# linnanwang/FastGen

Hardware: AMD Instinct MI355X
Metric: images/sec at 4-step distilled (DMD2) sampling (higher is better)
Workload: dtype fp32 (tensors, accumulate) with split-bf16 x3 MFMA conv products; 1 GPU; EDM CIFAR-10 32x32 SongUNet (55.7M params) DMD2 4-step 'sde' sampling, batch=512 per GPU; global_batch=512, sample_steps=4, parallelism=replicas x1 (no data-path collective), graph=True

## Files before the change

fastgen_amd/_lib.py:

```python
import ctypes
import os
from ctypes import POINTER, c_char_p, c_double, c_float, c_int, c_int64, c_size_t, c_uint64, c_void_p

_HERE = os.path.dirname(os.path.abspath(__file__))
LIB_PATH = os.path.join(_HERE, "libfastgen_amd.so")

FG_MAX_LEVELS = 8
FG_DTYPE_F32, FG_DTYPE_BF16, FG_DTYPE_BF16X3 = 0, 1, 2
DTYPE_NAMES = {"fp32": FG_DTYPE_F32, "bf16": FG_DTYPE_BF16, "bf16x3": FG_DTYPE_BF16X3}
FG_SAMPLE_SDE, FG_SAMPLE_ODE = 0, 1
FG_LOOP_X0, FG_LOOP_MEANFLOW, FG_LOOP_EULER = 0, 1, 2
FG_SCHEDULE_EDM, FG_SCHEDULE_RF = 0, 1
FG_DROP_PRECOND_INPUT, FG_DROP_PRECOND_OUTPUT = 1, 2
FG_BWD_DECODER, FG_BWD_ENCODER, FG_BWD_EMBED = 1, 2, 4
FG_MODEL_SONGUNET, FG_MODEL_DHARIWAL = 0, 1


class fg_edm_config(ctypes.Structure):
    _fields_ = [
        ("img_resolution", c_int), ("img_channels", c_int), ("label_dim", c_int), ("augment_dim", c_int),
        ("model_channels", c_int), ("num_levels", c_int), ("channel_mult", c_int * FG_MAX_LEVELS),
        ("channel_mult_emb", c_int), ("num_blocks", c_int), ("num_attn_resolutions", c_int),
        ("attn_resolutions", c_int * FG_MAX_LEVELS), ("channel_mult_noise", c_int), ("sigma_data", c_double),
        ("sigma_shift", c_double), ("compute_dtype", c_int), ("r_timestep", c_int), ("drop_precond", c_int),
# ... 9 lines not shown
        ("concat_balance", c_double), ("res_balance", c_double), ("attn_balance", c_double), ("clip_act", c_double),
        ("sigma_data", c_double), ("sigma_shift", c_double), ("compute_dtype", c_int), ("drop_precond", c_int),
    ]


class fg_dit_config(ctypes.Structure):
    _fields_ = [("input_size", c_int), ("patch_size", c_int), ("in_channels", c_int), ("hidden_size", c_int), ("depth", c_int),
                ("num_heads", c_int), ("mlp_hidden", c_int), ("embedding_rows", c_int), ("r_timestep", c_int), ("compute_dtype", c_int)]


class fg_wan_config(ctypes.Structure):
    _fields_ = [("num_heads", c_int), ("head_dim", c_int), ("in_channels", c_int), ("out_channels", c_int), ("text_dim", c_int),
                ("freq_dim", c_int), ("ffn_dim", c_int), ("num_layers", c_int), ("rope_max_seq_len", c_int), ("chunk_size", c_int),
                ("total_num_frames", c_int), ("eps", c_float)]


class fg_dit_sampler_config(ctypes.Structure):
    _fields_ = [("t_scale", c_double), ("guidance_scale", c_double), ("use_sit_convention", c_int), ("time_cond_diff", c_int),
                ("net_pred_flow", c_int), ("schedule", c_int)]


class fg_wan_sampler_config(ctypes.Structure):
    _fields_ = [("t_scale", c_double), ("context_noise", c_double), ("net_pred_flow", c_int), ("schedule", c_int), ("prefill_frames", c_int)]


SIGNATURES = {
    "fg_last_error": (c_char_p, []),
    "fg_version": (c_char_p, []),
    "fg_edm_create": (c_int, [POINTER(fg_edm_config), POINTER(c_void_p)]),
    "fg_edm_destroy": (None, [c_void_p]),
    "fg_edm_num_params": (c_int, [c_void_p]),
    "fg_edm_param_info": (c_int, [c_void_p, c_int, POINTER(c_char_p), POINTER(c_int), POINTER(c_int64)]),
    "fg_edm_bind_param": (c_int, [c_void_p, c_char_p, c_void_p, c_int64]),
    "fg_edm_pack_weights": (c_int, [c_void_p, c_void_p]),
    "fg_edm_workspace_bytes": (c_size_t, [c_void_p, c_int]),
    "fg_edm_forward": (c_int, [c_void_p, c_void_p, c_void_p, c_void_p, c_void_p, c_void_p, c_void_p, c_int, c_void_p,
                               c_size_t, c_void_p]),
    "fg_edm_num_feature_taps": (c_int, [c_void_p]),
    "fg_edm_feature_info": (c_int, [c_void_p, c_int, POINTER(c_char_p), POINTER(c_int), POINTER(c_int)]),
    "fg_edm_forward_features": (c_int, [c_void_p, c_void_p, c_void_p, c_void_p, c_void_p, c_void_p, POINTER(c_void_p), c_int,
                                        c_void_p, c_size_t, c_void_p]),
    "fg_sampler_run": (c_int, [c_void_p, c_void_p, c_void_p, POINTER(c_double), c_int, c_int, c_int, c_void_p, c_uint64,
                               c_void_p, c_int, c_void_p, c_size_t, c_int, c_void_p]),
    "fg_edm_t_list": (c_int, [c_int, POINTER(c_double)]),
    "fg_rf_t_list": (c_int, [c_int, POINTER(c_double)]),
    "fg_edm_profile_begin": (c_int, [c_void_p]),
    "fg_edm_profile_end": (c_int, [c_void_p, POINTER(c_int64), POINTER(c_double), POINTER(c_double)]),
    "fg_edm_num_blocks": (c_int, [c_void_p]),
    "fg_edm_block_info": (c_int, [c_void_p, c_int, POINTER(c_char_p), POINTER(c_int), POINTER(c_int), POINTER(c_int),
                                  POINTER(c_int), POINTER(c_int)]),
    "fg_edm_run_block": (c_int, [c_void_p, c_int, c_void_p, c_int, c_void_p, c_int, c_void_p, c_void_p, c_int, c_void_p,
                                 c_size_t, c_void_p]),
    "fg_op_gn_coeffs": (c_int, [c_void_p, c_int, c_void_p, c_int, c_void_p, c_void_p, c_float, c_void_p, c_int, c_int, c_void_p]),
    "fg_op_adm_conv_pack_bytes": (c_size_t, [c_int, c_int, c_int, c_int]),
    "fg_op_adm_conv_pack": (c_int, [c_int, c_void_p, c_void_p, c_int, c_int, c_int, c_void_p]),
    "fg_op_adm_conv": (c_int, [c_int, c_int, c_void_p, c_int, c_void_p, c_int, c_int, c_int, c_int, c_int, c_void_p, c_int, c_void_p,
                               c_void_p, c_void_p, c_int, c_void_p, c_int, c_void_p]),
    "fg_op_adm_gn_workspace_bytes": (c_size_t, [c_int, c_int, c_int]),
    "fg_op_adm_gn_coeffs": (c_int, [c_void_p, c_int, c_void_p, c_int, c_void_p, c_void_p, c_float, c_void_p, c_int, c_void_p, c_int,
                                    c_int, c_void_p, c_size_t, c_void_p]),
    "fg_op_adm_attention": (c_int, [c_void_p, c_void_p, c_int, c_int, c_int, c_void_p]),
    "fg_op_adm_map_in": (c_int, [c_void_p, c_void_p, c_void_p, c_void_p, c_int, c_void_p, c_int, c_int, c_void_p]),
    "fg_op_latents": (c_int, [c_void_p, c_double, c_void_p, c_int64, c_void_p]),
    "fg_op_forward_process": (c_int, [c_void_p, c_void_p, c_double, c_int, c_void_p, c_int64, c_void_p]),
    "fg_op_x0_to_eps": (c_int, [c_void_p, c_void_p, c_double, c_int, c_void_p, c_int64, c_void_p]),
    "fg_op_conv_wgrad_workspace_bytes": (ctypes.c_size_t, [c_int, c_int, c_int, c_int, c_int]),
    "fg_op_conv_wgrad": (c_int, [c_void_p, c_void_p, c_void_p, c_int, c_int, c_int, c_int, c_int, c_int, c_void_p, ctypes.c_size_t, c_void_p]),
    "fg_op_conv_wgrad_f32": (c_int, [c_void_p, c_void_p, c_void_p, c_int, c_int, c_int, c_int, c_int, c_int, c_void_p, ctypes.c_size_t, c_void_p]),
    "fg_edm_bind_grad": (c_int, [c_void_p, c_char_p, c_void_p, c_int64]),
    "fg_edm_block_backward_workspace_bytes": (c_size_t, [c_void_p, c_int, c_int]),
    "fg_edm_run_block_backward": (c_int, [c_void_p, c_int, c_void_p, c_int, c_void_p, c_int, c_void_p, c_void_p, c_void_p,
                                          c_void_p, c_void_p, c_int, c_void_p, c_size_t, c_void_p]),
    "fg_edm_backward_workspace_bytes": (c_size_t, [c_void_p, c_int]),
    "fg_edm_backward": (c_int, [c_void_p, c_void_p, c_void_p, c_void_p, c_void_p, c_void_p, c_void_p, c_int, c_int, c_void_p,
                                c_size_t, c_void_p]),
    "fg_edm_forward_train": (c_int, [c_void_p, c_void_p, c_void_p, c_void_p, c_void_p, c_void_p, c_void_p, c_int, c_void_p,
                                     c_size_t, c_void_p]),
    "fg_edm_backward_ex": (c_int, [c_void_p, c_void_p, c_void_p, c_void_p, c_void_p, c_void_p, c_void_p, c_void_p, c_void_p, c_int,
                                   c_int, c_void_p, c_size_t, c_void_p]),
    "fg_edm_backward_part": (c_int, [c_void_p, c_void_p, c_void_p, c_void_p, c_void_p, c_void_p, c_void_p, c_void_p, c_void_p, c_int,
                                     c_int, c_int, c_void_p, c_size_t, c_void_p]),
    "fg_edm2_create": (c_int, [POINTER(fg_edm2_config), POINTER(c_void_p)]),
    "fg_edm2_destroy": (None, [c_void_p]),
    "fg_edm2_num_params": (c_int, [c_void_p]),
    "fg_edm2_param_info": (c_int, [c_void_p, c_int, POINTER(c_char_p), POINTER(c_int), POINTER(c_int64)]),
    "fg_edm2_bind_param": (c_int, [c_void_p, c_char_p, c_void_p, c_int64]),
    "fg_edm2_pack_weights": (c_int, [c_void_p, c_void_p]),
    "fg_edm2_workspace_bytes": (c_size_t, [c_void_p, c_int]),
    "fg_edm2_forward": (c_int, [c_void_p, c_void_p, c_void_p, c_void_p, c_void_p, c_void_p, c_int, c_void_p, c_size_t, c_void_p]),
    "fg_edm2_set_training": (c_int, [c_void_p, c_int]),
    "fg_edm2_sampler_run": (c_int, [c_void_p, c_void_p, c_void_p, POINTER(c_double), c_int, c_int, c_int, c_void_p, c_uint64,
                                    c_void_p, c_int, c_void_p, c_size_t, c_int, c_void_p]),
    "fg_edm2_num_blocks": (c_int, [c_void_p]),
    "fg_edm2_block_info": (c_int, [c_void_p, c_int, POINTER(c_char_p), POINTER(c_int), POINTER(c_int), POINTER(c_int),
                                   POINTER(c_int), POINTER(c_int)]),
    "fg_edm2_run_block": (c_int, [c_void_p, c_int, c_void_p, c_int, c_void_p, c_int, c_void_p, c_void_p, c_int, c_void_p,
                                  c_size_t, c_void_p]),
    "fg_dit_create": (c_int, [POINTER(fg_dit_config), POINTER(c_void_p)]),
    "fg_dit_destroy": (None, [c_void_p]),
    "fg_dit_num_params": (c_int, [c_void_p]),
    "fg_dit_param_info": (c_int, [c_void_p, c_int, POINTER(c_char_p), POINTER(c_int), POINTER(c_int64)]),
    "fg_dit_bind_param": (c_int, [c_void_p, c_char_p, c_void_p, c_int64]),
    "fg_dit_pack_weights": (c_int, [c_void_p, c_void_p]),
    "fg_dit_pack_group": (c_int, [c_void_p, c_char_p, c_char_p, c_void_p]),
    "fg_dit_workspace_bytes": (c_size_t, [c_void_p, c_int]),
    "fg_dit_forward": (c_int, [c_void_p, c_void_p, c_void_p, c_void_p, c_void_p, c_void_p, c_void_p, c_int, c_void_p, c_size_t, c_void_p]),
# ... 66 lines not shown
```

fastgen_amd/csrc/conv.h:

```cpp
#pragma once
#include <hip/hip_runtime.h>

struct ConvArgs {
    const void* src1;
    const void* src2;
    int C1, C2;
    int Hs, Ws;
    int H, W;
    int B;
    const float2* ab;
    const void* wpack;
    const void* wpack_ws;
    const float* bias;
    const float* temb;
    int temb_stride;
    const void* resid;
    float scale;
    void* out;
    int Cout;
    float2* stats;
    int dbg;
    void* q_out;
    void* k_out;
    void* vt_out;
    const float* gate = nullptr;
    int gate_stride = 0;
    int act = 0;
    int heads = 0, head_dim = 0;
    size_t heads_lo_off = 0;
};

enum { PRO_NONE = 0, PRO_GN = 1, PRO_GN_SILU = 2 };
enum { RES_NONE = 0, RES_DOWN = 1, RES_UP = 2 };
enum { OUT_NHWC = 0, OUT_QKV = 1, OUT_TOK = 2, OUT_HEADS = 3 };

int launch_conv_fused(int dtype, int ks, int pro, int res, int outmode, const ConvArgs& a, hipStream_t stream);
int conv_stat_slots(int W);
bool conv_ws_supported(int dtype, int ks, int pro, int res, int outmode, const ConvArgs& a);
bool conv_ws_enabled();
int launch_conv_ws(int res, const ConvArgs& a, hipStream_t stream, bool prepare_only, int pro = PRO_GN_SILU);
bool conv_ws_shape_ok(int dtype, int cout, int cin, int res);
int launch_pack_conv_weights_ws(const float* w_oihw, void* wpack_ws, int cout, int cin, hipStream_t stream);
bool conv_x3ws_supported(int ks, int pro, int res, int outmode, const ConvArgs& a);
bool conv_x3ws_shape_ok(int cout, int cin, int res);
int conv_x3ws_stat_slots(int W);
int launch_conv_x3ws(int res, const ConvArgs& a, hipStream_t stream, bool prepare_only, int pro = PRO_GN_SILU);
int launch_pack_conv_weights_x3ws(const float* w_oihw, void* wpack_ws, int cout, int cin, hipStream_t stream);
int conv_launch_stat_slots(int dtype, int ks, int pro, int res, int outmode, const ConvArgs& a);
int launch_conv_ws_debug(const ConvArgs& a, int abl, hipStream_t stream);
int launch_conv_debug(int dtype, const ConvArgs& a, hipStream_t stream);
int conv_prepare_all(int dtype);
size_t conv_pack_elems(int cout, int cin, int ks);
int launch_pack_conv_weights(int dtype, const float* w_oihw, void* wpack, int cout, int cin, int ks, int qkv_perm,
                             hipStream_t stream);
```

fastgen_amd/csrc/conv.hip:

```cpp
#include "common.h"
#include "conv.h"
#include <stdlib.h>

#include <type_traits>

namespace {

constexpr int PITCH = 144;
constexpr int NTHR = 256;

template <int KS, int LOGW>
struct Geom {
    static constexpr int W = 1 << LOGW;
    static constexpr int LOGTW = (LOGW == 5) ? 4 : LOGW;
    static constexpr int TW = 1 << LOGTW;
    static constexpr int LOGTH = 3;
    static constexpr int TH = 1 << LOGTH;
    static constexpr int IMGS = 128 / (TH * TW);
    static constexpr int TCOLS = W / TW;
    static constexpr int TPI = (IMGS > 1) ? 1 : (W / TH) * TCOLS;
    static constexpr int PAD = KS / 2;
    static constexpr int HW_ = TW + 2 * PAD;
    static constexpr int HH_ = TH + 2 * PAD;
    static constexpr int HALO_PIX = IMGS * HH_ * HW_;
// ... 527 lines not shown
        if (res == RES_UP) return launch_w<T, 3, PRO_GN_SILU, RES_UP, OUT_NHWC>(a, s);
    }
    if (ks == 3 && pro == PRO_NONE && res == RES_NONE) return launch_w<T, 3, PRO_NONE, RES_NONE, OUT_NHWC>(a, s);
    if (ks == 1 && pro == PRO_NONE) {
        if (res == RES_NONE) return launch_w<T, 1, PRO_NONE, RES_NONE, OUT_NHWC>(a, s);
        if (res == RES_DOWN) return launch_w<T, 1, PRO_NONE, RES_DOWN, OUT_NHWC>(a, s);
        if (res == RES_UP) return launch_w<T, 1, PRO_NONE, RES_UP, OUT_NHWC>(a, s);
    }
    return (int)hipErrorInvalidValue;
}

int dispatch_t(int dtype, int ks, int pro, int res, int outmode, const ConvArgs& a, hipStream_t s) {
    switch (dtype) {
        case 0: return launch_t<float>(ks, pro, res, outmode, a, s);
        case 1: return launch_t<__bf16>(ks, pro, res, outmode, a, s);
        case 2: return launch_t<bf16x3>(ks, pro, res, outmode, a, s);
    }
    return (int)hipErrorInvalidValue;
}

}

int launch_conv_debug(int dtype, const ConvArgs& a, hipStream_t stream) {
    if (dtype != 1 || a.W != 32) return (int)hipErrorInvalidValue;
    g_debug_extra_lds = (a.dbg & 16) ? 48 * 1024 : 0;
    switch (a.dbg & 15) {
        case 0: return launch_one<__bf16, 3, PRO_GN_SILU, RES_NONE, 5, OUT_NHWC, 0>(a, stream);
        case 1: return launch_one<__bf16, 3, PRO_GN_SILU, RES_NONE, 5, OUT_NHWC, 1>(a, stream);
        case 2: return launch_one<__bf16, 3, PRO_GN_SILU, RES_NONE, 5, OUT_NHWC, 2>(a, stream);
        case 3: return launch_one<__bf16, 3, PRO_GN_SILU, RES_NONE, 5, OUT_NHWC, 3>(a, stream);
        case 4: return launch_one<__bf16, 3, PRO_GN_SILU, RES_NONE, 5, OUT_NHWC, 4>(a, stream);
        case 5: return launch_one<__bf16, 3, PRO_GN_SILU, RES_NONE, 5, OUT_NHWC, 5>(a, stream);
        case 6: return launch_one<__bf16, 3, PRO_GN_SILU, RES_NONE, 5, OUT_NHWC, 6>(a, stream);
        case 7: return launch_one<__bf16, 3, PRO_GN_SILU, RES_NONE, 5, OUT_NHWC, 7>(a, stream);
    }
    return (int)hipErrorInvalidValue;
}

int launch_conv_fused(int dtype, int ks, int pro, int res, int outmode, const ConvArgs& a, hipStream_t stream) {
    const int kc = dtype == 1 ? DT<__bf16>::KC : DT<float>::KC;
    if (a.H != a.W || (a.W != 8 && a.W != 16 && a.W != 32)) return (int)hipErrorInvalidValue;
    const bool tok = outmode == OUT_TOK || outmode == OUT_HEADS;
    if ((a.C1 % kc) || (a.C2 % kc) || (a.Cout % (tok ? 64 : 256)) || a.B <= 0) return (int)hipErrorInvalidValue;
    if (outmode == OUT_HEADS && (a.heads <= 0 || (a.head_dim % 4) || a.Cout != 3 * a.heads * a.head_dim || ((a.heads * a.head_dim) % 64) ||
                                 !a.q_out || !a.k_out || !a.vt_out))
        return (int)hipErrorInvalidValue;
    if (res == RES_NONE && (a.Hs != a.H || a.Ws != a.W)) return (int)hipErrorInvalidValue;
    if (res == RES_DOWN && (a.Hs != 2 * a.H || a.Ws != 2 * a.W)) return (int)hipErrorInvalidValue;
    if (res == RES_UP && (2 * a.Hs != a.H || 2 * a.Ws != a.W)) return (int)hipErrorInvalidValue;
    if (pro != PRO_NONE && !a.ab) return (int)hipErrorInvalidValue;
    if (outmode == OUT_QKV && (a.Cout != 768 || a.W > 16)) return (int)hipErrorInvalidValue;
    if (conv_ws_enabled() && conv_ws_supported(dtype, ks, pro, res, outmode, a)) return launch_conv_ws(res, a, stream, false, pro);
    if (dtype == 2 && conv_ws_enabled() && conv_x3ws_supported(ks, pro, res, outmode, a)) return launch_conv_x3ws(res, a, stream, false, pro);
    return dispatch_t(dtype, ks, pro, res, outmode, a, stream);
}

bool conv_ws_enabled() {
    static const bool on = [] {
        const char* e = getenv("FASTGEN_AMD_CONV_WS");
        return !(e && e[0] == '0');
    }();
    return on;
}

int conv_launch_stat_slots(int dtype, int ks, int pro, int res, int outmode, const ConvArgs& a) {
    if (dtype == 2 && conv_ws_enabled() && conv_x3ws_supported(ks, pro, res, outmode, a)) return conv_x3ws_stat_slots(a.W);
    return conv_stat_slots(a.W);
}

int conv_stat_slots(int W) { return W == 32 ? Geom<3, 5>::TPI : (W == 16 ? Geom<3, 4>::TPI : Geom<3, 3>::TPI); }

int conv_prepare_all(int dtype) {
    g_prepare_only = true;
    int rc = 0;
    ConvArgs a{};
    a.B = 1;
    a.Cout = 256;
    const int ws[3] = {8, 16, 32};
    for (int wi = 0; wi < 3 && !rc; ++wi) {
        a.W = a.H = ws[wi];
        for (int res = 0; res < 3 && !rc; ++res) {
            if (res != RES_DOWN)
                rc = dispatch_t(dtype, 3, PRO_GN_SILU, res, OUT_NHWC, a, nullptr);
            if (!rc) rc = dispatch_t(dtype, 1, PRO_NONE, res, OUT_NHWC, a, nullptr);
        }
        if (!rc) rc = dispatch_t(dtype, 3, PRO_NONE, RES_NONE, OUT_NHWC, a, nullptr);
        if (!rc && a.W <= 16) rc = dispatch_t(dtype, 1, PRO_GN, RES_NONE, OUT_QKV, a, nullptr);
        if (!rc && a.W == 16) rc = dispatch_t(dtype, 1, PRO_NONE, RES_NONE, OUT_TOK, a, nullptr);
        if (!rc && a.W == 16) rc = dispatch_t(dtype, 1, PRO_NONE, RES_NONE, OUT_HEADS, a, nullptr);
    }
    g_prepare_only = false;
    if (!rc && dtype == 2) {
        ConvArgs w{};
        for (int res : {RES_NONE, RES_UP})
            for (int ww : {32, 16}) {
                w.W = w.H = ww;
                if (!rc) rc = launch_conv_x3ws(res, w, nullptr, true, PRO_GN_SILU);
                if (!rc && res == RES_NONE) rc = launch_conv_x3ws(res, w, nullptr, true, PRO_NONE);
            }
    }
    if (!rc && dtype == 1) {
        ConvArgs w{};
        for (int res : {RES_NONE, RES_UP}) {
            w.W = w.H = 32;
            if (!rc) rc = launch_conv_ws(res, w, nullptr, true);
            if (res == RES_NONE) {
                w.C1 = -128;
                if (!rc) rc = launch_conv_ws(res, w, nullptr, true);
                w.C1 = 0;
            }
            w.W = w.H = 16;
            if (!rc) rc = launch_conv_ws(res, w, nullptr, true);
        }
    }
    return rc;
}

size_t conv_pack_elems(int cout, int cin, int ks) { return (size_t)cout * cin * ks * ks; }

// ... 13 lines not shown
```

fastgen_amd/csrc/engine.hip:

```cpp
#include <hip/hip_runtime.h>

#include <cmath>
#include <cstdarg>
#include <cstdio>
#include <cstdlib>
#include <cstring>
#include <string>
#include <map>
#include <vector>

#include "../../include/fastgen_amd.h"
#include "common.h"
#include "adm.h"
#include "edm2.h"
#include "conv.h"
#include "misc.h"

namespace {

thread_local std::string g_err;

int fail(int code, const char* fmt, ...) {
    char buf[512];
    va_list ap;
// ... 1183 lines not shown
}

int fg_edm_run_block(fg_edm* h, int index, const float* x1, int c1, const float* x2, int c2, const float* emb, float* out,
                     int batch, void* workspace, size_t workspace_bytes, void* stream) {
    if (!h || !x1 || !emb || !out) return fail(FG_EINVAL, "null argument");
    if (h->adm) return adm_run_block(h, index, x1, c1, x2, c2, emb, out, batch, workspace, workspace_bytes, (hipStream_t)stream);
    if (!h->packed) return fail(FG_ENOTREADY, "weights are not packed (call fg_edm_pack_weights)");
    if (index < 0 || index >= (int)h->blocks.size()) return fail(FG_EINVAL, "block index out of range");
    Workspace w;
    int rc0 = setup_ws(plan_workspace, h, batch, workspace, workspace_bytes, w);
    if (rc0) return rc0;
    hipStream_t s = (hipStream_t)stream;
    HIP_TRY(launch_linear(emb, h->aff_w, h->aff_b, w.temb, batch, h->emb_ch, h->temb_total, 0, s));
    const Block& b = *h->blocks[index];
    const size_t npix_in = (size_t)batch * b.res_in * b.res_in, npix_out = (size_t)batch * b.res_out * b.res_out;
    Act a1, a2;
    HIP_TRY(launch_to_act(h->dtype, x1, w.cvt1, (int64_t)npix_in * c1, s));
    a1.p = w.cvt1;
    if (c2) {
        HIP_TRY(launch_to_act(h->dtype, x2, w.cvt2, (int64_t)npix_in * c2, s));
        a2.p = w.cvt2;
    }
    int rc = run_block(h, b, a1, c1, a2, c2, w.temb, w.xa, batch, w, s);
    if (rc) return rc;
    HIP_TRY(launch_from_act(h->dtype, w.xa.p, out, (int64_t)npix_out * b.cout, s));
    return FG_OK;
}

#include "engine_train.inc"
#include "engine_dit.inc"
#include "engine_wan.inc"
#include "engine_sampler.inc"
#include "engine_edm2.inc"

int fg_op_gn_coeffs(const float* x1, int c1, const float* x2, int c2, const float* gamma, const float* beta, float eps,
                    float* ab_out, int batch, int hw, void* stream) {
    if (!x1 || !gamma || !beta || !ab_out) return fail(FG_EINVAL, "null argument");
    HIP_TRY(launch_gn_coeffs(0, x1, c1, c2 ? x2 : nullptr, c2, gamma, beta, eps, (float2*)ab_out, batch, hw, (hipStream_t)stream));
    return FG_OK;
}

size_t fg_op_adm_conv_pack_bytes(int mode, int cout, int cin, int ks) {
    if ((mode != FG_DTYPE_BF16 && mode != FG_DTYPE_BF16X3) || (ks != 1 && ks != 3) || cout <= 0 || cin <= 0 || cin % 32) return 0;
    return adm_conv_pack_elems(mode, cout, cin, ks) * sizeof(__bf16);
}
int fg_op_adm_conv_pack(int mode, const float* w_oihw, void* packed, int cout, int cin, int ks, void* stream) {
    if (!fg_op_adm_conv_pack_bytes(mode, cout, cin, ks))
        return fail(FG_EINVAL, "fg_op_adm_conv_pack: mode %d (1 bf16, 2 bf16x3), ks %d (1, 3), cout %d > 0, cin %d (multiple of 32)", mode,
                    ks, cout, cin);
    if (!w_oihw || !packed) return fail(FG_EINVAL, "fg_op_adm_conv_pack: null pointer");
    HIP_TRY(adm_pack_conv_weights(mode, w_oihw, packed, cout, cin, ks, (hipStream_t)stream));
    return FG_OK;
}
int fg_op_adm_conv(int mode, int ks, const float* src1, int c1, const float* src2, int c2, int batch, int hs, int h, int res_mode,
                   const float* ab, int silu, const void* packed, const float* bias, const float* resid, int resid_mode, float* out,
                   int cout, void* stream) {
    if ((mode != FG_DTYPE_BF16 && mode != FG_DTYPE_BF16X3) || (ks != 1 && ks != 3))
        return fail(FG_EINVAL, "fg_op_adm_conv: mode %d (1 bf16, 2 bf16x3), ks %d (1, 3)", mode, ks);
    if (c1 <= 0 || c1 % 32 || c2 < 0 || c2 % 32 || cout <= 0 || batch <= 0 || batch > 65535)
        return fail(FG_EINVAL, "fg_op_adm_conv: c1 %d > 0 and c2 %d >= 0 multiples of 32, cout %d > 0, batch %d in 1 .. 65535", c1, c2,
                    cout, batch);
    const bool res_ok = (res_mode == 0 && hs == h) || (res_mode == 1 && hs == 2 * h) || (res_mode == 2 && h == 2 * hs);
    if (h <= 0 || h > 4096 || !res_ok) return fail(FG_EINVAL, "fg_op_adm_conv: res_mode %d with hs %d, h %d", res_mode, hs, h);
    if (resid && (resid_mode < 0 || resid_mode > 2 || (resid_mode == 2 && h % 2)))
        return fail(FG_EINVAL, "fg_op_adm_conv: resid_mode %d (0, 1, 2 with h even) at h %d", resid_mode, h);
    if (!src1 || (c2 && !src2) || !packed || !out) return fail(FG_EINVAL, "fg_op_adm_conv: null pointer");
    if (((uintptr_t)src1 | (uintptr_t)(c2 ? src2 : nullptr) | (uintptr_t)packed) & 15 || (uintptr_t)ab & 7)
        return fail(FG_EINVAL, "fg_op_adm_conv: src1 / src2 / packed must be 16-byte aligned, ab 8-byte aligned");
    AdmConvArgs a;
    a.src1 = src1, a.src2 = c2 ? src2 : nullptr, a.C1 = c1, a.C2 = c2, a.Hs = hs, a.H = h, a.B = batch, a.res_mode = res_mode;
    a.ab = (const float2*)ab, a.silu = silu ? 1 : 0, a.w = packed, a.bias = bias, a.resid = resid, a.resid_mode = resid ? resid_mode : 0;
    a.out = out, a.Cout = cout;
    HIP_TRY(adm_launch_conv(mode, ks, a, (hipStream_t)stream));
    return FG_OK;
}
size_t fg_op_adm_gn_workspace_bytes(int batch, int hw, int c) {
    if (batch <= 0 || hw <= 0 || c <= 0) return 0;
    return adm_gn_part_elems(batch, hw, c) * sizeof(float2);
}
int fg_op_adm_gn_coeffs(const float* x1, int c1, const float* x2, int c2, const float* gamma, const float* beta, float eps,
                        const float* temb, int temb_stride, float* ab_out, int batch, int hw, void* workspace, size_t workspace_bytes,
                        void* stream) {
    const int C = c1 + c2;
    if (c1 <= 0 || c1 % 2 || c2 < 0 || c2 % 2 || C < 8)
        return fail(FG_EINVAL, "fg_op_adm_gn_coeffs: c1 %d > 0 and c2 %d >= 0 must be even, c1 + c2 >= 8", c1, c2);
    const int G = std::min(32, C / 4);
    if (C % G || (C / G) % 2)
        return fail(FG_EINVAL, "fg_op_adm_gn_coeffs: %d channels in %d groups: the group size must be a whole, even number", C, G);
    if (batch <= 0 || batch > 65535 || hw <= 0 || hw > (1 << 22))
        return fail(FG_EINVAL, "fg_op_adm_gn_coeffs: batch %d (1 .. 65535), hw %d (1 .. 2^22)", batch, hw);
    if (temb && temb_stride < 2 * C) return fail(FG_EINVAL, "fg_op_adm_gn_coeffs: temb_stride %d < 2 C = %d", temb_stride, 2 * C);
    if (!x1 || (c2 && !x2) || !gamma || !beta || !ab_out || !workspace) return fail(FG_EINVAL, "fg_op_adm_gn_coeffs: null pointer");
    if (((uintptr_t)x1 | (uintptr_t)(c2 ? x2 : nullptr) | (uintptr_t)ab_out | (uintptr_t)workspace) & 7)
        return fail(FG_EINVAL, "fg_op_adm_gn_coeffs: x1 / x2 / ab_out / workspace must be 8-byte aligned");
    const size_t need = fg_op_adm_gn_workspace_bytes(batch, hw, C);
    if (workspace_bytes < need)
        return fail(FG_EINVAL, "fg_op_adm_gn_coeffs: workspace too small (%zu < %zu bytes)", workspace_bytes, need);
    HIP_TRY(adm_launch_gn(x1, c1, c2 ? x2 : nullptr, c2, gamma, beta, eps, temb, temb_stride, (float2*)workspace, (float2*)ab_out, batch,
                          hw, (hipStream_t)stream));
    return FG_OK;
}
int fg_op_adm_attention(const float* qkv, float* out, int batch, int t, int heads, void* stream) {
    if (t <= 0 || t % 64 || heads <= 0 || heads > 65535 || batch <= 0 || batch > 65535)
        return fail(FG_EINVAL, "fg_op_adm_attention: t %d (a positive multiple of 64), heads %d, batch %d (1 .. 65535)", t, heads, batch);
    if (!qkv || !out) return fail(FG_EINVAL, "fg_op_adm_attention: null pointer");
    HIP_TRY(adm_launch_attention(qkv, out, batch, t, heads, (hipStream_t)stream));
// ... 178 lines not shown
```

include/fastgen_amd.h:

```cpp
#ifndef FASTGEN_AMD_H
#define FASTGEN_AMD_H

#include <stddef.h>
#include <stdint.h>

#ifdef __cplusplus
extern "C" {
#endif

#define FG_API __attribute__((visibility("default")))

#define FG_OK 0
#define FG_EINVAL 1
#define FG_ENOTREADY 2
#define FG_EHIP 3
#define FG_ENOMEM 4

#define FG_DTYPE_F32 0
#define FG_DTYPE_BF16 1
#define FG_DTYPE_BF16X3 2

#define FG_SAMPLE_SDE 0
#define FG_SAMPLE_ODE 1

// ... 28 lines not shown
    double sigma_data;
    double sigma_shift;
    int compute_dtype;
    int r_timestep;
    int drop_precond;
    int schedule;
    int model_type;
} fg_edm_config;

typedef struct fg_edm fg_edm;

FG_API const char* fg_last_error(void);
FG_API const char* fg_version(void);

FG_API int fg_edm_create(const fg_edm_config* cfg, fg_edm** out);
FG_API void fg_edm_destroy(fg_edm* h);

FG_API int fg_edm_num_params(const fg_edm* h);
FG_API int fg_edm_param_info(const fg_edm* h, int index, const char** name, int* ndim, int64_t shape[4]);

FG_API int fg_edm_bind_param(fg_edm* h, const char* name, const float* device_ptr, int64_t numel);
FG_API int fg_edm_pack_weights(fg_edm* h, void* stream);

FG_API size_t fg_edm_workspace_bytes(const fg_edm* h, int batch);

FG_API int fg_edm_forward(fg_edm* h, const float* x_t, const double* t, const double* r, const float* class_labels, float* out,
                   float* emb_out, int batch, void* workspace, size_t workspace_bytes, void* stream);

FG_API int fg_edm_num_feature_taps(const fg_edm* h);
FG_API int fg_edm_feature_info(const fg_edm* h, int index, const char** key, int* channels, int* resolution);
FG_API int fg_edm_forward_features(fg_edm* h, const float* x_t, const double* t, const double* r, const float* class_labels,
                            float* out, float* const* features, int batch, void* workspace, size_t workspace_bytes,
                            void* stream);

FG_API int fg_sampler_run(fg_edm* h, const float* noise, const float* class_labels, const double* t_list, int steps,
                   int sample_type, int loop_kind, const float* eps, uint64_t seed, float* out, int batch,
                   void* workspace, size_t workspace_bytes, int use_graph, void* stream);

FG_API int fg_edm_t_list(int sample_steps, double* out_host);
FG_API int fg_rf_t_list(int sample_steps, double* out_host);

FG_API int fg_edm_profile_begin(fg_edm* h);
FG_API int fg_edm_profile_end(fg_edm* h, int64_t* launches, double* total_ms, double* total_flops);


FG_API int fg_edm_num_blocks(const fg_edm* h);
FG_API int fg_edm_block_info(const fg_edm* h, int index, const char** key, int* cin, int* cout, int* res_in, int* res_out,
                      int* has_attention);
FG_API int fg_edm_run_block(fg_edm* h, int index, const float* x1, int c1, const float* x2, int c2, const float* emb,
                     float* out, int batch, void* workspace, size_t workspace_bytes, void* stream);

FG_API int fg_op_gn_coeffs(const float* x1, int c1, const float* x2, int c2, const float* gamma, const float* beta,
                    float eps, float* ab_out, int batch, int hw, void* stream);

FG_API size_t fg_op_adm_conv_pack_bytes(int mode, int cout, int cin, int ks);
FG_API int fg_op_adm_conv_pack(int mode, const float* w_oihw, void* packed, int cout, int cin, int ks, void* stream);
FG_API int fg_op_adm_conv(int mode, int ks, const float* src1, int c1, const float* src2, int c2, int batch, int hs, int h,
                          int res_mode, const float* ab, int silu, const void* packed, const float* bias, const float* resid,
                          int resid_mode, float* out, int cout, void* stream);
FG_API size_t fg_op_adm_gn_workspace_bytes(int batch, int hw, int c);
FG_API int fg_op_adm_gn_coeffs(const float* x1, int c1, const float* x2, int c2, const float* gamma, const float* beta, float eps,
                               const float* temb, int temb_stride, float* ab_out, int batch, int hw, void* workspace,
                               size_t workspace_bytes, void* stream);
FG_API int fg_op_adm_attention(const float* qkv, float* out, int batch, int t, int heads, void* stream);
FG_API int fg_op_adm_map_in(const float* c_noise, const float* freqs, const float* aug, const float* wa, int aug_dim, float* out,
                            int batch, int n, void* stream);

FG_API int fg_op_latents(const float* noise, double t_init, float* out, int64_t total, void* stream);
FG_API int fg_op_forward_process(const float* x0, const float* eps, double t, int schedule, float* out, int64_t total,
                          void* stream);
FG_API int fg_op_x0_to_eps(const float* xt, const float* x0, double t, int schedule, float* out, int64_t total, void* stream);
FG_API size_t fg_op_conv_wgrad_workspace_bytes(int batch, int res, int cin, int cout, int ks);
FG_API int fg_op_conv_wgrad(const void* act, const void* dy, float* dw, int batch, int res, int cin, int cout, int ks,
                     int accumulate, void* workspace, size_t workspace_bytes, void* stream);

FG_API int fg_op_conv_wgrad_f32(const float* act, const float* dy, float* dw, int batch, int res, int cin, int cout, int ks,
                                int accumulate, void* workspace, size_t workspace_bytes, void* stream);

FG_API int fg_edm_bind_grad(fg_edm* h, const char* name, float* grad, int64_t numel);
FG_API size_t fg_edm_block_backward_workspace_bytes(const fg_edm* h, int index, int batch);
FG_API int fg_edm_run_block_backward(fg_edm* h, int index, const float* x1, int c1, const float* x2, int c2, const float* emb,
                              const float* dout, float* dx1, float* dx2, float* demb, int batch, void* workspace,
                              size_t workspace_bytes, void* stream);

FG_API size_t fg_edm_backward_workspace_bytes(const fg_edm* h, int batch);
FG_API int fg_edm_backward(fg_edm* h, const float* x_t, const double* t, const double* r, const float* labels, const float* dout,
                    float* out, int have_forward, int batch, void* workspace, size_t workspace_bytes, void* stream);
FG_API int fg_edm_forward_train(fg_edm* h, const float* x_t, const double* t, const double* r, const float* labels, float* out,
                         float* const* features, int batch, void* workspace, size_t workspace_bytes, void* stream);
FG_API int fg_edm_backward_ex(fg_edm* h, const float* x_t, const double* t, const double* r, const float* labels, const float* dout,
                       const float* const* dfeatures, float* out, float* dx_t, int have_forward, int batch, void* workspace,
                       size_t workspace_bytes, void* stream);

#define FG_BWD_DECODER 1
#define FG_BWD_ENCODER 2
#define FG_BWD_EMBED 4
FG_API int fg_edm_backward_part(fg_edm* h, const float* x_t, const double* t, const double* r, const float* labels, const float* dout,
                                const float* const* dfeatures, float* out, float* dx_t, int have_forward, int parts, int batch,
                                void* workspace, size_t workspace_bytes, void* stream);

FG_API int fg_disc_edm_num_params(int res);
FG_API size_t fg_disc_edm_workspace_bytes(int res, int batch);
FG_API int fg_disc_edm_run(const float* feat, int res, const float* const* params, float* logits, const float* dlogits, float* dfeat,
                    float* const* grads, int batch, void* workspace, size_t workspace_bytes, void* stream);

FG_API int fg_edm_jvp(fg_edm* h, const float* x_t, const double* t, const double* r, const float* labels, const float* vx, const float* vt,
// ... 153 lines not shown
```

Before: 2685 img/s.

## Add dedicated bf16x3 pointwise 1x1 conv kernel for skip and QKV projections

Adds a specialised 1x1-convolution kernel for the split-bf16x3 path. Each block computes 256 output channels, uses double-buffered LDS A tiles with register-prefetched weights, and fuses down/up resampling, the GN prologue for QKV, and a bias/temb/residual/stats epilogue. It is dispatched ahead of the generic template path whenever the shape is supported and is on by default through an environment switch. The aim is to stop running 1x1 convs through the general 3x3-oriented kernel and its weaker reuse, at the cost of more code and higher register and LDS pressure. It also exposes a new C API for the op.

New measurement: 2696 img/s (median of 6 runs). Within noise of the previous version (+0.4%).

```diff
diff --git a/fastgen_amd/_lib.py b/fastgen_amd/_lib.py
--- a/fastgen_amd/_lib.py
+++ b/fastgen_amd/_lib.py
@@ -85,6 +85,11 @@
     "fg_edm_run_block": (c_int, [c_void_p, c_int, c_void_p, c_int, c_void_p, c_int, c_void_p, c_void_p, c_int, c_void_p,
                                  c_size_t, c_void_p]),
     "fg_op_gn_coeffs": (c_int, [c_void_p, c_int, c_void_p, c_int, c_void_p, c_void_p, c_float, c_void_p, c_int, c_int, c_void_p]),
+    "fg_op_conv1x1_x3_pack_bytes": (c_size_t, [c_int, c_int]),
+    "fg_op_conv1x1_x3_pack": (c_int, [c_void_p, c_void_p, c_int, c_int, c_int, c_void_p]),
+    "fg_op_conv1x1_x3": (c_int, [c_void_p, c_int, c_void_p, c_int, c_int, c_int, c_int, c_int, c_void_p, c_void_p, c_void_p, c_void_p,
+                                 c_int, c_void_p, c_float, c_void_p, c_void_p, c_void_p, c_void_p, c_int, c_void_p, POINTER(c_int),
+                                 c_void_p]),
     "fg_op_adm_conv_pack_bytes": (c_size_t, [c_int, c_int, c_int, c_int]),
     "fg_op_adm_conv_pack": (c_int, [c_int, c_void_p, c_void_p, c_int, c_int, c_int, c_void_p]),
     "fg_op_adm_conv": (c_int, [c_int, c_int, c_void_p, c_int, c_void_p, c_int, c_int, c_int, c_int, c_int, c_void_p, c_int, c_void_p,
diff --git a/fastgen_amd/csrc/conv.h b/fastgen_amd/csrc/conv.h
--- a/fastgen_amd/csrc/conv.h
+++ b/fastgen_amd/csrc/conv.h
@@ -46,6 +46,10 @@
 int conv_x3ws_stat_slots(int W);
 int launch_conv_x3ws(int res, const ConvArgs& a, hipStream_t stream, bool prepare_only, int pro = PRO_GN_SILU);
 int launch_pack_conv_weights_x3ws(const float* w_oihw, void* wpack_ws, int cout, int cin, hipStream_t stream);
+bool conv_pw_enabled();
+bool conv_pw3_supported(int ks, int pro, int res, int outmode, const ConvArgs& a);
+int conv_pw3_stat_slots(int W);
+int launch_conv_pw3(int pro, int res, int outmode, const ConvArgs& a, hipStream_t stream);
 int conv_launch_stat_slots(int dtype, int ks, int pro, int res, int outmode, const ConvArgs& a);
 int launch_conv_ws_debug(const ConvArgs& a, int abl, hipStream_t stream);
 int launch_conv_debug(int dtype, const ConvArgs& a, hipStream_t stream);
diff --git a/fastgen_amd/csrc/conv.hip b/fastgen_amd/csrc/conv.hip
--- a/fastgen_amd/csrc/conv.hip
+++ b/fastgen_amd/csrc/conv.hip
@@ -603,6 +603,7 @@
     if (outmode == OUT_QKV && (a.Cout != 768 || a.W > 16)) return (int)hipErrorInvalidValue;
     if (conv_ws_enabled() && conv_ws_supported(dtype, ks, pro, res, outmode, a)) return launch_conv_ws(res, a, stream, false, pro);
     if (dtype == 2 && conv_ws_enabled() && conv_x3ws_supported(ks, pro, res, outmode, a)) return launch_conv_x3ws(res, a, stream, false, pro);
+    if (dtype == 2 && ks == 1 && conv_pw_enabled() && conv_pw3_supported(ks, pro, res, outmode, a)) return launch_conv_pw3(pro, res, outmode, a, stream);
     return dispatch_t(dtype, ks, pro, res, outmode, a, stream);
 }
 
@@ -616,6 +617,7 @@
 
 int conv_launch_stat_slots(int dtype, int ks, int pro, int res, int outmode, const ConvArgs& a) {
     if (dtype == 2 && conv_ws_enabled() && conv_x3ws_supported(ks, pro, res, outmode, a)) return conv_x3ws_stat_slots(a.W);
+    if (dtype == 2 && ks == 1 && conv_pw_enabled() && conv_pw3_supported(ks, pro, res, outmode, a)) return conv_pw3_stat_slots(a.W);
     return conv_stat_slots(a.W);
 }
 
diff --git a/fastgen_amd/csrc/conv_pw3.hip b/fastgen_amd/csrc/conv_pw3.hip
--- /dev/null
+++ b/fastgen_amd/csrc/conv_pw3.hip
@@ -0,0 +1,358 @@
+#include "common.h"
+#include "conv.h"
+#include <stdlib.h>
+
+#include <type_traits>
+
+namespace {
+
+constexpr int PW_NTHR = 256;
+constexpr int PW_PITCH = 144;
+constexpr int PW_KC = DT<bf16x3>::KC;
+constexpr int PW_KK = PW_KC / 16;
+constexpr int PW_NT = 2;
+constexpr int PW_ABUF = 128 * PW_PITCH;
+constexpr int PW_WFRAG = 512 * DT<bf16x3>::WPARTS;
+constexpr int PW_ABMAX = 512;
+
+template <int LOGW>
+struct PwGeom {
+    static constexpr int W = 1 << LOGW;
+    static constexpr int LOGTW = (LOGW == 5) ? 4 : LOGW;
+    static constexpr int TW = 1 << LOGTW;
+    static constexpr int LOGTH = 3;
+    static constexpr int TH = 1 << LOGTH;
+    static constexpr int IMGS = 128 / (TH * TW);
+    static constexpr int TCOLS = W / TW;
+    static constexpr int TPI = (IMGS > 1) ? 1 : (W / TH) * TCOLS;
+};
+
+template <int PRO>
+__device__ __forceinline__ float pw_pro(float x, float2 ab) {
+    return fmaf(x, ab.x, ab.y);
+}
+
+template <int PRO, int RES, int LOGW, int OUTMODE>
+__global__ __launch_bounds__(PW_NTHR, 2) void conv_pw3_kernel(const ConvArgs a, const int ncb) {
+    using G = PwGeom<LOGW>;
+    constexpr int ND = (RES == RES_DOWN) ? 4 : 1;
+    constexpr int DIST = (RES == RES_DOWN) ? 1 : 2;
+    constexpr int WSETS = DIST;
+    constexpr int NITEMS = 2;
+    constexpr int PSTRIDE = 64;
+    constexpr int NAB = (PRO == PRO_NONE) ? 0 : G::IMGS;
+
+    __shared__ __attribute__((aligned(16))) char smem[2 * PW_ABUF];
+
+    const int tid = threadIdx.x;
+    const int lane = tid & 63;
+    const int wave = __builtin_amdgcn_readfirstlane(tid >> 6);
+    const int r = lane & 31, h = lane >> 5;
+    const int tile = blockIdx.x / ncb, nblk = blockIdx.x - tile * ncb;
+    const int Cin = a.C1 + a.C2;
+    const int nchunk = Cin / PW_KC;
+    const int H = a.H;
+
+    const int n_base = (G::IMGS > 1) ? tile * G::IMGS : tile / G::TPI;
+    const int slot = (G::IMGS > 1) ? 0 : tile % G::TPI;
+    const int row0 = (slot / G::TCOLS) * G::TH, col0 = (slot % G::TCOLS) * G::TW;
+
+    const int wst = nchunk * (PW_KK * PW_WFRAG);
+    const __amdgpu_buffer_rsrc_t wrs = make_rsrc(reinterpret_cast<const __bf16*>(a.wpack) + (size_t)(nblk * (4 * PW_NT) + wave * PW_NT) * wst);
+    const int wlane = lane * 8;
+
+    const float* src1 = reinterpret_cast<const float*>(a.src1);
+    const float* src2 = reinterpret_cast<const float*>(a.src2);
+
+    const int oct = tid & 3;
+    const int hq0 = tid >> 2;
+    int it_sp[NITEMS];
+    bool it_ok[NITEMS];
+#pragma unroll
+    for (int i = 0; i < NITEMS; ++i) {
+        const int p = hq0 + i * PSTRIDE;
+        const int n = n_base + (p >> (G::LOGTW + G::LOGTH));
+        const int y = row0 + ((p >> G::LOGTW) & (G::TH - 1));
+        const int x = col0 + (p & (G::TW - 1));
+        const int sy = (RES == RES_DOWN) ? 2 * y : ((RES == RES_UP) ? (y >> 1) : y);
+        const int sx = (RES == RES_DOWN) ? 2 * x : ((RES == RES_UP) ? (x >> 1) : x);
+        it_ok[i] = n < a.B;
+        it_sp[i] = (min(n, a.B - 1) * a.Hs + sy) * a.Ws + sx;
+    }
+
+    __shared__ __attribute__((aligned(16))) float2 ab_lds[NAB > 0 ? NAB * PW_ABMAX : 1];
+    if constexpr (NAB > 0) {
+        for (int e = tid; e < NAB * Cin; e += PW_NTHR) {
+            const int im = e / Cin, c = e - im * Cin;
+            ab_lds[e] = a.ab[(size_t)min(n_base + im, a.B - 1) * Cin + c];
+        }
+        __syncthreads();
+    }
+
+    Frag8<float> raw[DIST][NITEMS][ND];
+    Frag8<bf16x3> bw[WSETS][PW_NT][PW_KK];
+
+    auto load_w = [&](int chunk, Frag8<bf16x3> (&b)[PW_NT][PW_KK]) {
+#pragma unroll
+        for (int nt = 0; nt < PW_NT; ++nt)
+#pragma unroll
+            for (int kk = 0; kk < PW_KK; ++kk) load_frag_rsrc(b[nt][kk], wrs, wlane, chunk * (PW_KK * PW_WFRAG) + nt * wst + kk * PW_WFRAG);
+    };
+    auto load_a = [&](int chunk, Frag8<float> (&rw)[NITEMS][ND]) {
+        const int c0 = chunk * PW_KC + oct * 8;
+        const bool first = c0 < a.C1;
+        const float* sb = first ? src1 + c0 : src2 + (c0 - a.C1);
+        const int cs = first ? a.C1 : a.C2;
+#pragma unroll
+        for (int i = 0; i < NITEMS; ++i)
+#pragma unroll
+            for (int d = 0; d < ND; ++d) {
+                const int sp = it_sp[i] + ((RES == RES_DOWN) ? (d >> 1) * a.Ws + (d & 1) : 0);
+                rw[i][d] = load_frag(sb + (size_t)sp * cs);
+            }
+    };
+    auto stage = [&](int chunk, char* abuf, const Frag8<float> (&rw)[NITEMS][ND]) {
+#pragma unroll
+        for (int i = 0; i < NITEMS; ++i) {
+            const int p = hq0 + i * PSTRIDE;
+            float o[8];
+#pragma unroll
+            for (int j = 0; j < 8; ++j) o[j] = 0.f;
+#pragma unroll
+            for (int d = 0; d < ND; ++d) {
+                float v[8];
+                widen8(rw[i][d], v);
+                if (G::IMGS > 1) {
+#pragma unroll
+                    for (int j = 0; j < 8; ++j) v[j] = it_ok[i] ? v[j] : 0.f;
+                }
+                if constexpr (NAB > 0) {
+                    const int im = (NAB > 1) ? (p >> (G::LOGTW + G::LOGTH)) : 0;
+                    const f32x4* q = reinterpret_cast<const f32x4*>(ab_lds + im * Cin + chunk * PW_KC + oct * 8);
+#pragma unroll
+                    for (int j = 0; j < 8; j += 2) {
+                        const f32x4 c = q[j / 2];
+                        o[j] += it_ok[i] ? pw_pro<PRO>(v[j], make_float2(c[0], c[1])) : 0.f;
+                        o[j + 1] += it_ok[i] ? pw_pro<PRO>(v[j + 1], make_float2(c[2], c[3])) : 0.f;
+                    }
+                } else {
+#pragma unroll
+                    for (int j = 0; j < 8; ++j) o[j] += v[j];
+                }
+            }
+            if (ND == 4) {
+#pragma unroll
+                for (int j = 0; j < 8; ++j) o[j] *= 0.25f;
+            }
+            lds_store_a<bf16x3>(abuf + p * PW_PITCH + oct * 16, o);
+        }
+    };
+
+    f32x16 acc[4][PW_NT];
+#pragma unroll
+    for (int mt = 0; mt < 4; ++mt)
+#pragma unroll
+        for (int nt = 0; nt < PW_NT; ++nt)
+#pragma unroll
+            for (int i = 0; i < 16; ++i) acc[mt][nt][i] = 0.f;
+
+    load_w(0, bw[0]);
+#pragma unroll
+    for (int s = 0; s < DIST; ++s) load_a(min(s, nchunk - 1), raw[s]);
+    stage(0, smem, raw[0]);
+    __syncthreads();
+
+    const int lane_off = r * PW_PITCH + h * 16;
+    auto body = [&](const int chunk, auto par) {
+        constexpr int P = decltype(par)::value;
+        constexpr int SN = (DIST == 2) ? P : 0;
+        constexpr int SS = (DIST == 2) ? 1 - P : 0;
+        constexpr int WC = (WSETS == 2) ? P : 0;
+        const int last = nchunk - 1;
+        const int wnext = min(chunk + 1, last);
+        if constexpr (WSETS == 2) load_w(wnext, bw[1 - WC]);
+        load_a(min(chunk + DIST, last), raw[SN]);
+        __builtin_amdgcn_sched_barrier(0);
+        const char* abase = smem + P * PW_ABUF + lane_off;
+#pragma unroll
+        for (int kk = 0; kk < PW_KK; ++kk) {
+#pragma unroll
+            for (int mt = 0; mt < 4; ++mt) {
+                const Frag8<bf16x3> af = lds_read_a<bf16x3>(abase + mt * 32 * PW_PITCH, kk);
+#pragma unroll
+                for (int nt = 0; nt < PW_NT; ++nt) mma16(acc[mt][nt], af, bw[WC][nt][kk]);
+            }
+            if constexpr (WSETS == 1) {
+#pragma unroll
+                for (int nt = 0; nt < PW_NT; ++nt)
+                    load_frag_rsrc(bw[0][nt][kk], wrs, wlane, wnext * (PW_KK * PW_WFRAG) + nt * wst + kk * PW_WFRAG);
+            }
+            __builtin_amdgcn_sched_barrier(0);
+        }
+        stage(min(chunk + 1, last), smem + (1 - P) * PW_ABUF, raw[SS]);
+        __syncthreads();
+    };
+    for (int chunk = 0; chunk < nchunk; chunk += 2) {
+        body(chunk, std::integral_constant<int, 0>{});
+        body(chunk + 1, std::integral_constant<int, 1>{});
+    }
+
+    const int HWo = H * G::W;
+    if (OUTMODE == OUT_NHWC || nblk < 2) {
+        constexpr int QPW = 8 * PW_NT;
+        constexpr int RP = 64 / QPW;
+        constexpr int NP = 32 / RP;
+        constexpr int EP_PITCH = 32 * PW_NT * 4 + 16;
+        constexpr int MT_PER_IMG = 4 / G::IMGS;
+        static_assert(4 * 32 * EP_PITCH <= 2 * PW_ABUF, "epilogue scratch must fit in the A buffers");
+        char* ep = smem + wave * (32 * EP_PITCH);
+        const int c4 = lane % QPW, prow = lane / QPW;
+        const int co0 = nblk * (128 * PW_NT) + wave * (32 * PW_NT) + c4 * 4;
+        const bool qk = (OUTMODE == OUT_QKV);
+        float* out = reinterpret_cast<float*>(qk ? (nblk == 0 ? a.q_out : a.k_out) : a.out);
+        const float* resid = qk ? nullptr : reinterpret_cast<const float*>(a.resid);
+        const int ostride = qk ? 256 : a.Cout;
+        const int co_out = qk ? co0 - nblk * 256 : co0;
+        f32x4 bias4 = {0.f, 0.f, 0.f, 0.f};
+        if (a.bias) bias4 = *reinterpret_cast<const f32x4*>(a.bias + co0);
+        float ssum[G::IMGS], ssq[G::IMGS];
+#pragma unroll
+        for (int im = 0; im < G::IMGS; ++im) ssum[im] = ssq[im] = 0.f;
+        auto goff = [&](int mt, int j, bool& ok) -> size_t {
+            const int p = mt * 32 + j * RP + prow;
+            const int x = col0 + (p & (G::TW - 1));
+            const int y = row0 + ((p >> G::LOGTW) & (G::TH - 1));
+            const int n = n_base + mt / MT_PER_IMG;
+            ok = n < a.B;
+            return (((size_t)n * H + y) * G::W + x) * ostride + co_out;
+        };
+        f32x4 rcur[NP], rnext[NP];
+        auto issue_resid = [&](int mt, f32x4 (&rr)[NP]) {
+#pragma unroll
+            for (int j = 0; j < NP; ++j) {
+                bool ok;
+                const size_t go = goff(mt, j, ok);
+                rr[j] = f32x4{};
+                if (ok) rr[j] = raw_load4(resid + go);
+            }
+        };
+        if (resid) issue_resid(0, rcur);
+#pragma unroll
+        for (int mt = 0; mt < 4; ++mt) {
+            const int im = mt / MT_PER_IMG;
+            const int n = n_base + im;
+            if (resid && mt + 1 < 4) issue_resid(mt + 1, rnext);
+#pragma unroll
+            for (int nt = 0; nt < PW_NT; ++nt)
+#pragma unroll
+                for (int i = 0; i < 16; ++i)
+                    *reinterpret_cast<float*>(ep + acc_row(i, h) * EP_PITCH + (nt * 32 + r) * 4) = acc[mt][nt][i];
+            f32x4 add = bias4;
+            if (!qk && a.temb && n < a.B) add += *reinterpret_cast<const f32x4*>(a.temb + (size_t)n * a.temb_stride + co0);
+#pragma unroll
+            for (int j = 0; j < NP; ++j) {
+                const int pl = j * RP + prow;
+                f32x4 v = *reinterpret_cast<const f32x4*>(ep + pl * EP_PITCH + c4 * 16);
+                bool ok;
+                const size_t go = goff(mt, j, ok);
+                if (ok) {
+                    v += add;
+                    if (resid) v += rcur[j];
+                    v *= a.scale;
+                    const f32x4 vr = store4(out + go, v);
+                    ssum[im] += (vr[0] + vr[1]) + (vr[2] + vr[3]);
+                    ssq[im] += (vr[0] * vr[0] + vr[1] * vr[1]) + (vr[2] * vr[2] + vr[3] * vr[3]);
+                }
+            }
+#pragma unroll
+            for (int j = 0; j < NP; ++j) rcur[j] = rnext[j];
+        }
+        if (!qk && a.stats) {
+#pragma unroll
+            for (int im = 0; im < G::IMGS; ++im) {
+                float sv = ssum[im], qv = ssq[im];
+#pragma unroll
+                for (int sh = QPW; sh < 64; sh <<= 1) {
+                    sv += __shfl_xor(sv, sh);
+                    qv += __shfl_xor(qv, sh);
+                }
+                const int n = n_base + im;
+                if (prow == 0 && n < a.B)
+                    a.stats[((size_t)n * G::TPI + slot) * (a.Cout >> 2) + (co0 >> 2)] = make_float2(sv, qv);
+            }
+        }
+    } else {
+        float* vt = reinterpret_cast<float*>(a.vt_out);
+#pragma unroll
+        for (int nt = 0; nt < PW_NT; ++nt) {
+            const int cl = wave * 64 + nt * 32 + r;
+            const float bias = a.bias ? a.bias[nblk * 256 + cl] : 0.f;
+#pragma unroll
+            for (int mt = 0; mt < 4; ++mt) {
+#pragma unroll
+                for (int i4 = 0; i4 < 16; i4 += 4) {
+                    const int p = mt * 32 + acc_row(i4, h);
+                    const int x = col0 + (p & (G::TW - 1));
+                    const int y = row0 + ((p >> G::LOGTW) & (G::TH - 1));
+                    const int n = n_base + (p >> (G::LOGTW + G::LOGTH));
+                    if (n < a.B) {
+                        const size_t vo = ((size_t)n * 256 + cl) * HWo + y * G::W + x;
+                        const f32x4 vv = {acc[mt][nt][i4] + bias, acc[mt][nt][i4 + 1] + bias, acc[mt][nt][i4 + 2] + bias,
+                                          acc[mt][nt][i4 + 3] + bias};
+                        store4(vt + vo, vv);
+                    }
+                }
+            }
+        }
+    }
+}
+
+template <int PRO, int RES, int LOGW, int OUTMODE>
+int pw3_launch_one(const ConvArgs& a, hipStream_t stream) {
+    using G = PwGeom<LOGW>;
+    const int tiles = (G::IMGS > 1) ? (a.B + G::IMGS - 1) / G::IMGS : a.B * G::TPI;
+    const int ncb = a.Cout / 256;
+    hipLaunchKernelGGL((conv_pw3_kernel<PRO, RES, LOGW, OUTMODE>), dim3(tiles * ncb), dim3(PW_NTHR), 0, stream, a, ncb);
+    return (int)hipGetLastError();
+}
+
+template <int PRO, int RES, int OUTMODE>
+int pw3_launch_w(const ConvArgs& a, hipStream_t s) {
+    switch (a.W) {
+        case 32: return pw3_launch_one<PRO, RES, 5, OUTMODE>(a, s);
+        case 16: return pw3_launch_one<PRO, RES, 4, OUTMODE>(a, s);
+        case 8: return pw3_launch_one<PRO, RES, 3, OUTMODE>(a, s);
+    }
+    return (int)hipErrorInvalidValue;
+}
+
+}
+
+bool conv_pw_enabled() {
+    static const bool on = [] {
+        const char* e = getenv("FASTGEN_AMD_CONV_PW");
+        return !(e && e[0] == '0');
+    }();
+    return on;
+}
+
+bool conv_pw3_supported(int ks, int pro, int res, int outmode, const ConvArgs& a) {
+    if (ks != 1 || a.H != a.W || (a.W != 8 && a.W != 16 && a.W != 32) || a.B <= 0) return false;
+    if ((a.C1 % PW_KC) || (a.C2 % PW_KC) || a.C1 + a.C2 <= 0 || ((a.C1 + a.C2) % (2 * PW_KC)) || (a.Cout % 256) || !a.wpack) return false;
+    if (a.C2 && !a.src2) return false;
+    if (outmode == OUT_QKV) return pro == PRO_GN && res == RES_NONE && a.C1 + a.C2 <= PW_ABMAX && a.Cout == 768 && a.W <= 16 && a.ab && a.q_out && a.k_out && a.vt_out;
+    if (outmode != OUT_NHWC || pro != PRO_NONE) return false;
+    if (res == RES_NONE) return a.Hs == a.H && a.Ws == a.W;
+    if (res == RES_DOWN) return a.Hs == 2 * a.H && a.Ws == 2 * a.W;
+    if (res == RES_UP) return 2 * a.Hs == a.H && 2 * a.Ws == a.W;
+    return false;
+}
+
+int conv_pw3_stat_slots(int W) { return W == 32 ? PwGeom<5>::TPI : (W == 16 ? PwGeom<4>::TPI : PwGeom<3>::TPI); }
+
+int launch_conv_pw3(int pro, int res, int outmode, const ConvArgs& a, hipStream_t stream) {
+    if (outmode == OUT_QKV) return pw3_launch_w<PRO_GN, RES_NONE, OUT_QKV>(a, stream);
+    if (res == RES_DOWN) return pw3_launch_w<PRO_NONE, RES_DOWN, OUT_NHWC>(a, stream);
+    if (res == RES_UP) return pw3_launch_w<PRO_NONE, RES_UP, OUT_NHWC>(a, stream);
+    return pw3_launch_w<PRO_NONE, RES_NONE, OUT_NHWC>(a, stream);
+}
diff --git a/fastgen_amd/csrc/engine.hip b/fastgen_amd/csrc/engine.hip
--- a/fastgen_amd/csrc/engine.hip
+++ b/fastgen_amd/csrc/engine.hip
@@ -1259,6 +1259,39 @@
     HIP_TRY(adm_pack_conv_weights(mode, w_oihw, packed, cout, cin, ks, (hipStream_t)stream));
     return FG_OK;
 }
+size_t fg_op_conv1x1_x3_pack_bytes(int cout, int cin) {
+    if (cout <= 0 || cin <= 0 || cout % 256 || cin % 32) return 0;
+    return conv_pack_elems(cout, cin, 1) * 2 * sizeof(uint16_t);
+}
+int fg_op_conv1x1_x3_pack(const float* w, void* packed, int cout, int cin, int qkv_perm, void* stream) {
+    if (!fg_op_conv1x1_x3_pack_bytes(cout, cin) || !w || !packed || (qkv_perm && cout != 768))
+        return fail(FG_EINVAL, "fg_op_conv1x1_x3_pack: cout %d (multiple of 256; 768 with qkv_perm), cin %d (multiple of 32)", cout, cin);
+    HIP_TRY(launch_pack_conv_weights(FG_DTYPE_BF16X3, w, packed, cout, cin, 1, qkv_perm ? 1 : 0, (hipStream_t)stream));
+    return FG_OK;
+}
+int fg_op_conv1x1_x3(const float* src1, int c1, const float* src2, int c2, int batch, int hs, int h, int res_mode, const float* ab,
+                     const void* packed, const float* bias, const float* temb, int temb_stride, const float* resid, float scale, float* out,
+                     float* q, float* k, float* vt, int cout, float* stats, int* stat_slots, void* stream) {
+    const bool qkv = q != nullptr;
+    if (c1 <= 0 || c1 % 32 || c2 < 0 || c2 % 32 || cout <= 0 || cout % 256 || batch <= 0 || (h != 8 && h != 16 && h != 32))
+        return fail(FG_EINVAL, "fg_op_conv1x1_x3: c1 %d, c2 %d (multiples of 32), cout %d (of 256), batch %d, h %d (8, 16, 32)", c1, c2,
+                    cout, batch, h);
+    const bool res_ok = (res_mode == 0 && hs == h) || (res_mode == 1 && hs == 2 * h) || (res_mode == 2 && h == 2 * hs);
+    if (!res_ok) return fail(FG_EINVAL, "fg_op_conv1x1_x3: res_mode %d with hs %d, h %d", res_mode, hs, h);
+    if (!src1 || (c2 && !src2) || !packed || (!qkv && !out) || (qkv && (!k || !vt || !ab || res_mode || cout != 768 || h > 16)))
+        return fail(FG_EINVAL, "fg_op_conv1x1_x3: null pointer, or a qkv call without ab / at res_mode %d, cout %d, h %d", res_mode, cout, h);
+    if (((uintptr_t)src1 | (uintptr_t)(c2 ? src2 : nullptr) | (uintptr_t)packed | (uintptr_t)out | (uintptr_t)resid | (uintptr_t)ab) & 15)
+        return fail(FG_EINVAL, "fg_op_conv1x1_x3: tensors must be 16-byte aligned");
+    ConvArgs a{};
+    a.src1 = src1, a.src2 = c2 ? src2 : nullptr, a.C1 = c1, a.C2 = c2, a.Hs = a.Ws = hs, a.H = a.W = h, a.B = batch;
+    a.ab = (const float2*)ab, a.wpack = packed, a.bias = bias, a.temb = temb, a.temb_stride = temb_stride;
+    a.resid = qkv ? nullptr : resid, a.scale = qkv ? 1.f : scale, a.out = qkv ? nullptr : out, a.Cout = cout;
+    a.stats = qkv ? nullptr : (float2*)stats, a.q_out = q, a.k_out = k, a.vt_out = vt;
+    const int pro = ab ? PRO_GN : PRO_NONE, outmode = qkv ? OUT_QKV : OUT_NHWC;
+    if (stat_slots) *stat_slots = conv_launch_stat_slots(FG_DTYPE_BF16X3, 1, pro, res_mode, outmode, a);
+    HIP_TRY(launch_conv_fused(FG_DTYPE_BF16X3, 1, pro, res_mode, outmode, a, (hipStream_t)stream));
+    return FG_OK;
+}
 int fg_op_adm_conv(int mode, int ks, const float* src1, int c1, const float* src2, int c2, int batch, int hs, int h, int res_mode,
                    const float* ab, int silu, const void* packed, const float* bias, const float* resid, int resid_mode, float* out,
                    int cout, void* stream) {
diff --git a/include/fastgen_amd.h b/include/fastgen_amd.h
--- a/include/fastgen_amd.h
+++ b/include/fastgen_amd.h
@@ -104,6 +104,13 @@
 
 FG_API int fg_op_gn_coeffs(const float* x1, int c1, const float* x2, int c2, const float* gamma, const float* beta,
                     float eps, float* ab_out, int batch, int hw, void* stream);
+
+FG_API size_t fg_op_conv1x1_x3_pack_bytes(int cout, int cin);
+FG_API int fg_op_conv1x1_x3_pack(const float* w_oi, void* packed, int cout, int cin, int qkv_perm, void* stream);
+FG_API int fg_op_conv1x1_x3(const float* src1, int c1, const float* src2, int c2, int batch, int hs, int h, int res_mode,
+                            const float* ab, const void* packed, const float* bias, const float* temb, int temb_stride,
+                            const float* resid, float scale, float* out, float* q, float* k, float* vt, int cout, float* stats,
+                            int* stat_slots, void* stream);
 
 FG_API size_t fg_op_adm_conv_pack_bytes(int mode, int cout, int cin, int ks);
 FG_API int fg_op_adm_conv_pack(int mode, const float* w_oihw, void* packed, int cout, int cin, int ks, void* stream);
```
